# shenyunhang/APE

Hardware: AMD Instinct MI355X
Metric: images/sec @1024^2 APE-L_D fwd (higher is better)
Workload: dtype bf16

## Files before the change

ape_amd/csrc/select.hip:

```cpp
#include "common.h"
#include "../../include/ape_hip.h"

__device__ __forceinline__ bool iou_gt(const float4 a, const float4 b, float thr) {
  const float area_a = (a.z - a.x) * (a.w - a.y);
  const float area_b = (b.z - b.x) * (b.w - b.y);
  const float xx1 = fmaxf(a.x, b.x), yy1 = fmaxf(a.y, b.y);
  const float xx2 = fminf(a.z, b.z), yy2 = fminf(a.w, b.w);
  const float w = fmaxf(0.f, xx2 - xx1), h = fmaxf(0.f, yy2 - yy1);
  const float inter = w * h;
  return inter / (area_a + area_b - inter) > thr;
}

__global__ __launch_bounds__(64) void nms_mask_kernel(const float4* __restrict__ boxes, const int* __restrict__ groups, int n,
                                                      float thr, unsigned long long* __restrict__ mask, int nw) {
  __shared__ float4 cb[64];
  __shared__ int cg[64];
  const int rb = blockIdx.y, cbk = blockIdx.x, t = threadIdx.x;
  const int j0 = cbk * 64;
  if (j0 + t < n) {
    cb[t] = boxes[j0 + t];
    cg[t] = groups ? groups[j0 + t] : 0;
  }
  __syncthreads();
  const int i = rb * 64 + t;
  if (i >= n) return;
  const float4 bi = boxes[i];
  const int gi = groups ? groups[i] : 0;
  unsigned long long bits = 0ull;
  const int cnt = min(64, n - j0);
  for (int j = 0; j < cnt; ++j) {
    if (j0 + j != i && cg[j] == gi && iou_gt(bi, cb[j], thr)) bits |= (1ull << j);
  }
  mask[(size_t)i * nw + cbk] = bits;
}

__device__ __forceinline__ unsigned long long readlane64(unsigned long long v, int lane_uniform) {
  const unsigned lo = (unsigned)__builtin_amdgcn_readlane((int)(unsigned)(v & 0xffffffffull), lane_uniform);
  const unsigned hi = (unsigned)__builtin_amdgcn_readlane((int)(unsigned)(v >> 32), lane_uniform);
  return ((unsigned long long)hi << 32) | lo;
}

__device__ __forceinline__ unsigned long long uniform64(unsigned long long v) {
  const unsigned lo = (unsigned)__builtin_amdgcn_readfirstlane((int)(unsigned)(v & 0xffffffffull));
  const unsigned hi = (unsigned)__builtin_amdgcn_readfirstlane((int)(unsigned)(v >> 32));
  return ((unsigned long long)hi << 32) | lo;
}
__device__ __forceinline__ unsigned long long wave_or64(unsigned long long v) {
  unsigned lo = (unsigned)(v & 0xffffffffull), hi = (unsigned)(v >> 32);
#pragma unroll
  for (int o = 32; o > 0; o >>= 1) { lo |= (unsigned)__shfl_xor((int)lo, o, 64); hi |= (unsigned)__shfl_xor((int)hi, o, 64); }
  return ((unsigned long long)hi << 32) | lo;
}

template <bool USE_LDS>
__global__ __launch_bounds__(256) void nms_scan_segments_kernel(const unsigned long long* __restrict__ mask, int nw, int n,
                                                                const int* __restrict__ seg, const uint8_t* __restrict__ valid,
                                                                uint8_t* __restrict__ keep) {
  extern __shared__ __attribute__((aligned(16))) unsigned long long sub[];
  const int s0 = seg[blockIdx.x], s1 = seg[blockIdx.x + 1];
  if (s1 <= s0) return;
  const int w0 = s0 >> 6, w1 = (s1 - 1) >> 6;
  const int nws = w1 - w0 + 1;
  const int r_base = w0 * 64;
  if (USE_LDS) {
    const int nrows = (w1 + 1) * 64 - r_base;
    for (int e = threadIdx.x; e < nrows * nws; e += 256) {
      const int r = e / nws, w = e - r * nws;
      const int row = r_base + r;
      sub[e] = row < n ? mask[(size_t)row * nw + w0 + w] : 0ull;
    }
    __syncthreads();
  }
  if (threadIdx.x >= 64) return;
  const int lane = threadIdx.x;
  auto word = [&](int row, int c) -> unsigned long long {
    if (USE_LDS) return sub[(size_t)(row - r_base) * nws + (c - w0)];
    return mask[(size_t)(row < n ? row : n - 1) * nw + c];
  };
  unsigned long long kept0 = 0ull, kept1 = 0ull;
  for (int c = w0; c <= w1; ++c) {
    unsigned long long acc = 0ull;
    for (int cp = w0; cp < c; cp += 8) {
      unsigned long long t[8];
#pragma unroll
      for (int u = 0; u < 8; ++u) {
        const int cq = cp + u;
        const int cqc = cq < c ? cq : cp;
        const int rel = cqc - w0;
        const unsigned long long km = readlane64(rel >= 64 ? kept1 : kept0, rel & 63);
        const bool take = cq < c && ((km >> lane) & 1ull);
        const unsigned long long v = word(cqc * 64 + lane, c);
        t[u] = take ? v : 0ull;
      }
#pragma unroll
      for (int u = 0; u < 8; ++u) acc |= t[u];
    }
    const unsigned long long remc = uniform64(wave_or64(acc));
    const int i = c * 64 + lane;
    const bool in_seg = i >= s0 && i < s1;
    const bool ok = in_seg && (valid == nullptr || valid[i] != 0);
    const unsigned long long row_c = ok ? word(i, c) : 0ull;
    unsigned long long alive = __builtin_amdgcn_ballot_w64(ok) & ~remc;
    unsigned long long kept = 0ull;
    while (alive != 0ull) {
      const int j = __builtin_ctzll(alive);
      kept |= 1ull << j;
      alive &= ~(1ull << j);
      alive &= ~readlane64(row_c, j);
    }
    if (in_seg) keep[i] = (uint8_t)((kept >> lane) & 1ull);
    const int rel = c - w0;
    if (lane == (rel & 63)) { if (rel >= 64) kept1 = kept; else kept0 = kept; }
  }
}

__global__ __launch_bounds__(256) void nms_scan_classes_kernel(const unsigned long long* __restrict__ mask, int nw, int n,
                                                               const int* __restrict__ order, const uint8_t* __restrict__ valid,
                                                               uint8_t* __restrict__ keep, int num_classes) {
  extern __shared__ __attribute__((aligned(16))) unsigned long long smask[];
  const int tid = threadIdx.x, lane = tid & 63, wave = tid >> 6;
  for (int i = tid; i < n * nw; i += 256) smask[i] = mask[i];
  __syncthreads();
  const int c = blockIdx.x * 4 + wave;
  if (c >= num_classes) return;
  const int* ord = order + (size_t)c * n;
  unsigned long long rem = 0ull;
  for (int base = 0; base < n; base += 64) {
    const int p = base + lane;
    const int qv = p < n ? ord[p] : 0;
    const int okv = (p < n) && (valid == nullptr || valid[(size_t)c * n + p] != 0);
    int keptv = 0;
    const int cnt = min(64, n - base);
    for (int u = 0; u < cnt; ++u) {
      const int qi = __builtin_amdgcn_readlane(qv, u);
      const int ok = __builtin_amdgcn_readlane(okv, u);
      const unsigned long long row = lane < nw ? smask[(size_t)qi * nw + lane] : 0ull;
      const unsigned long long r = readlane64(rem, qi >> 6);
      const bool kept = ok && !((r >> (qi & 63)) & 1ull);
      if (kept) rem |= row;
      if (lane == u) keptv = kept ? 1 : 0;
    }
    if (p < n) keep[(size_t)c * n + p] = (uint8_t)keptv;
  }
}

extern "C" int ape_hip_nms_mask_words(int n) { return ceil_div(n, 64); }

extern "C" int ape_hip_nms_mask(const float* boxes, const int* groups, int n, float iou_thr, uint64_t* mask, void* stream) {
  APE_CHECK_ARG(boxes && mask && n > 0 && ((uintptr_t)boxes) % 16 == 0, "ape_hip_nms_mask: bad args");
  const int nw = ceil_div(n, 64);
  APE_LAUNCH(nms_mask_kernel, dim3(nw, nw), dim3(64), 0, (hipStream_t)stream, (const float4*)boxes, groups, n, iou_thr,
                     (unsigned long long*)mask, nw);
  APE_CHECK_LAUNCH("ape_hip_nms_mask");
  return 0;
}

extern "C" int ape_hip_nms_scan_segments(const uint64_t* mask, int n, const int* seg_offsets, int num_segments, int max_segment,
                                         const uint8_t* valid, uint8_t* keep, void* stream) {
  APE_CHECK_ARG(mask && seg_offsets && keep && n > 0 && num_segments > 0, "ape_hip_nms_scan_segments: bad args");
  APE_CHECK_ARG(max_segment <= 126 * 64, "ape_hip_nms_scan_segments: segment longer than %d candidates", 126 * 64);
  const size_t sub_rows = (size_t)(ceil_div(max_segment, 64) + 1) * 64, sub_words = (size_t)ceil_div(max_segment, 64) + 1;
  const size_t lds = sub_rows * sub_words * 8;
  if (lds <= 160 * 1024) {
    static ApeOncePerDevice attr_done;
    if (attr_done.first()) {
      (void)hipFuncSetAttribute((const void*)nms_scan_segments_kernel<true>, hipFuncAttributeMaxDynamicSharedMemorySize, 160 * 1024);
    }
    APE_LAUNCH(nms_scan_segments_kernel<true>, dim3(num_segments), dim3(256), lds, (hipStream_t)stream,
                       (const unsigned long long*)mask, ceil_div(n, 64), n, seg_offsets, valid, keep);
  } else {
    APE_LAUNCH(nms_scan_segments_kernel<false>, dim3(num_segments), dim3(256), 0, (hipStream_t)stream,
                       (const unsigned long long*)mask, ceil_div(n, 64), n, seg_offsets, valid, keep);
  }
  APE_CHECK_LAUNCH("ape_hip_nms_scan_segments");
  return 0;
}

extern "C" int ape_hip_nms_scan_classes(const uint64_t* mask, int n, const int* order, int num_classes, const uint8_t* valid,
                                        uint8_t* keep, void* stream) {
  const int nw = ceil_div(n, 64);
  const size_t lds = (size_t)n * nw * 8;
  APE_CHECK_ARG(mask && order && keep && n > 0 && num_classes > 0 && lds <= 160 * 1024,
                "ape_hip_nms_scan_classes: bad args (the n x n/64 bit matrix must fit the 160 KiB LDS: n <= 1280)");
  static ApeOncePerDevice attr_done;
  if (attr_done.first()) {
    (void)hipFuncSetAttribute((const void*)nms_scan_classes_kernel, hipFuncAttributeMaxDynamicSharedMemorySize, 160 * 1024);
  }
  APE_LAUNCH(nms_scan_classes_kernel, dim3(ceil_div(num_classes, 4)), dim3(256), lds, (hipStream_t)stream,
                     (const unsigned long long*)mask, nw, n, order, valid, keep, num_classes);
  APE_CHECK_LAUNCH("ape_hip_nms_scan_classes");
  return 0;
}
```

ape_amd/csrc/topk.hip:

```cpp
#include "common.h"
#include "../../include/ape_hip.h"

typedef unsigned long long u64;
#define TK_THREADS 1024

__device__ __forceinline__ uint32_t ordkey(float x) {
  const uint32_t u = __float_as_uint(x);
  return u ^ ((u >> 31) ? 0xffffffffu : 0x80000000u);
}
__device__ __forceinline__ float ordkey_inv(uint32_t k) {
  return __uint_as_float(k ^ ((k >> 31) ? 0x80000000u : 0xffffffffu));
}
__device__ __forceinline__ float sigmoid_f(float x) { return 1.f / (1.f + expf(-x)); }

struct TkLevels {
  int start[8];
  int n[8];
  int L;
};
__device__ __forceinline__ int level_of(const TkLevels& lv, int idx) {
  int l = 0;
#pragma unroll
  for (int i = 1; i < 8; ++i) l += (i < lv.L && idx >= lv.start[i]) ? 1 : 0;
  return l;
}

template <int N>
__device__ __forceinline__ void bitonic_desc(u64* s) {
  for (int k = 2; k <= N; k <<= 1) {
    for (int j = k >> 1; j > 0; j >>= 1) {
      for (int i = threadIdx.x; i < N; i += TK_THREADS) {
        const int p = i ^ j;
        if (p > i) {
          const u64 a = s[i], b = s[p];
          const bool first_larger = (i & k) == 0;
          if (first_larger ? (a < b) : (a > b)) { s[i] = b; s[p] = a; }
        }
      }
      __syncthreads();
    }
  }
}

template <typename KeyFn>
__device__ __forceinline__ void radix_select(KeyFn key, int n, int k, uint32_t* hist, uint32_t* sh, uint32_t& thr, uint32_t& rem) {
  uint32_t prefix = 0, r = (uint32_t)k;
  for (int shift = 24; shift >= 0; shift -= 8) {
    for (int b = threadIdx.x; b < 256; b += TK_THREADS) hist[b] = 0;
    __syncthreads();
    const uint32_t himask = shift == 24 ? 0u : (0xffffffffu << (shift + 8));
    for (int i0 = 0; i0 < n; i0 += TK_THREADS) {
      const int i = i0 + threadIdx.x;
      const uint32_t kk = i < n ? key(i) : 0u;
      bool live = i < n && (kk & himask) == prefix;
      const uint32_t bin = (kk >> shift) & 255u;
      u64 todo = __ballot(live);
      while (todo) {
        const int leader = __ffsll((long long)todo) - 1;
        const uint32_t lb = (uint32_t)__builtin_amdgcn_readlane((int)bin, leader);
        const u64 same = __ballot(live && bin == lb);
        if ((int)(threadIdx.x & 63) == leader) atomicAdd(&hist[lb], (uint32_t)__popcll(same));
        todo &= ~same;
        if (live && bin == lb) live = false;
      }
    }
    __syncthreads();
    if (threadIdx.x == 0) {
      uint32_t cum = 0;
      int b = 255;
      for (; b > 0; --b) {
        if (cum + hist[b] >= r) break;
        cum += hist[b];
      }
      sh[0] = prefix | ((uint32_t)b << shift);
      sh[1] = r - cum;
    }
    __syncthreads();
    prefix = sh[0];
    r = sh[1];
    __syncthreads();
  }
  thr = prefix;
  rem = r;
}

template <typename KeyFn, typename CompFn>
__device__ __forceinline__ void block_topk(KeyFn key, CompFn composite, int n, int k, u64* comp, uint32_t* hist, uint32_t* sh, uint32_t* wcnt) {
  comp[threadIdx.x] = 0ull;
  __syncthreads();
  if (n <= k) {
    for (int i = threadIdx.x; i < n; i += TK_THREADS) comp[i] = composite(i);
    __syncthreads();
  } else {
    uint32_t thr, rem;
    radix_select(key, n, k, hist, sh, thr, rem);
    const uint32_t ngt = (uint32_t)k - rem;
    const int lane = threadIdx.x & 63, wave = threadIdx.x >> 6;
    uint32_t base_gt = 0, base_eq = 0;
    for (int i0 = 0; i0 < n; i0 += TK_THREADS) {
      const int i = i0 + threadIdx.x;
      const uint32_t kk = i < n ? key(i) : 0u;
      const bool gt = i < n && kk > thr, eq = i < n && kk == thr;
      const u64 bg = __ballot(gt), be = __ballot(eq);
      const u64 lt = (1ull << lane) - 1ull;
      if (lane == 0) { wcnt[wave] = (uint32_t)__popcll(bg); wcnt[16 + wave] = (uint32_t)__popcll(be); }
      __syncthreads();
      uint32_t wg = 0, we = 0, tg = 0, te = 0;
#pragma unroll
      for (int w = 0; w < 16; ++w) {
        const uint32_t cg = wcnt[w], ce = wcnt[16 + w];
        if (w < wave) { wg += cg; we += ce; }
        tg += cg; te += ce;
      }
      if (gt) comp[base_gt + wg + (uint32_t)__popcll(bg & lt)] = composite(i);
      if (eq) {
        const uint32_t rank = base_eq + we + (uint32_t)__popcll(be & lt);
        if (rank < rem) comp[ngt + rank] = composite(i);
      }
      base_gt += tg;
      base_eq += te;
      __syncthreads();
    }
  }
  bitonic_desc<1024>(comp);
}

template <int PER>
__device__ __forceinline__ void block_topk_regs(const uint32_t (&kk)[PER], int n, int k, uint32_t gbase, u64* comp, uint32_t* hist,
                                                uint32_t* sh, uint32_t* wcnt) {
  comp[threadIdx.x] = 0ull;
  __syncthreads();
  const int lane = threadIdx.x & 63, wave = threadIdx.x >> 6;
  if (n <= k) {
    if ((int)threadIdx.x < n) comp[threadIdx.x] = ((u64)kk[0] << 32) | (u64)(0xffffffffu - (gbase + threadIdx.x));
    __syncthreads();
  } else {
    uint32_t prefix = 0, r = (uint32_t)k;
    for (int shift = 24; shift >= 0; shift -= 8) {
      for (int b = threadIdx.x; b < 256; b += TK_THREADS) hist[b] = 0;
      __syncthreads();
      const uint32_t himask = shift == 24 ? 0u : (0xffffffffu << (shift + 8));
#pragma unroll
      for (int j = 0; j < PER; ++j) {
        const int e = j * TK_THREADS + threadIdx.x;
        bool live = e < n && (kk[j] & himask) == prefix;
        const uint32_t bin = (kk[j] >> shift) & 255u;
        u64 todo = __ballot(live);
        while (todo) {
          const int leader = __ffsll((long long)todo) - 1;
          const uint32_t lb = (uint32_t)__builtin_amdgcn_readlane((int)bin, leader);
          const u64 same = __ballot(live && bin == lb);
          if (lane == leader) atomicAdd(&hist[lb], (uint32_t)__popcll(same));
          todo &= ~same;
          if (live && bin == lb) live = false;
        }
      }
      __syncthreads();
      if (threadIdx.x == 0) {
        uint32_t cum = 0;
        int b = 255;
        for (; b > 0; --b) {
          if (cum + hist[b] >= r) break;
          cum += hist[b];
        }
        sh[0] = prefix | ((uint32_t)b << shift);
        sh[1] = r - cum;
      }
      __syncthreads();
      prefix = sh[0];
      r = sh[1];
      __syncthreads();
    }
    const uint32_t thr = prefix, rem = r, ngt = (uint32_t)k - rem;
    uint32_t base_gt = 0, base_eq = 0;
#pragma unroll
    for (int j = 0; j < PER; ++j) {
      const int e = j * TK_THREADS + threadIdx.x;
      const bool gt = e < n && kk[j] > thr, eq = e < n && kk[j] == thr;
      const u64 bg = __ballot(gt), be = __ballot(eq);
      const u64 lt = (1ull << lane) - 1ull;
      if (lane == 0) { wcnt[wave] = (uint32_t)__popcll(bg); wcnt[16 + wave] = (uint32_t)__popcll(be); }
      __syncthreads();
      uint32_t wg = 0, we = 0, tg = 0, te = 0;
#pragma unroll
      for (int w = 0; w < 16; ++w) {
        const uint32_t cg = wcnt[w], ce = wcnt[16 + w];
        if (w < wave) { wg += cg; we += ce; }
        tg += cg; te += ce;
      }
      const u64 c = ((u64)kk[j] << 32) | (u64)(0xffffffffu - (gbase + (uint32_t)e));
      if (gt) comp[base_gt + wg + (uint32_t)__popcll(bg & lt)] = c;
      if (eq) {
        const uint32_t rank = base_eq + we + (uint32_t)__popcll(be & lt);
        if (rank < rem) comp[ngt + rank] = c;
      }
      base_gt += tg;
      base_eq += te;
      __syncthreads();
    }
  }
  bitonic_desc<1024>(comp);
}

#define TK_STAGE2_MAX 12288
#define TK_MAX_JOBS 96
struct TkJobs {
  int njobs, nseg;
  int seg_first[8], seg_jobs[8], seg_k[8], seg_n[8], seg_mode[8];
  int start[TK_MAX_JOBS], n[TK_MAX_JOBS], seg[TK_MAX_JOBS];
};

__device__ __forceinline__ void stage2_gather(const u64* __restrict__ ws, int first_job, int njobs, int k, u64* lds) {
  const int m = njobs * k;
  for (int i = threadIdx.x; i < m; i += TK_THREADS) lds[i] = ws[(size_t)(first_job + i / k) * 1024 + (i % k)];
  __syncthreads();
}

__global__ __launch_bounds__(256) void enc_finalize_kernel(const float* __restrict__ cls2, const float* __restrict__ d,
                                                           const float* __restrict__ anchors, int T, float* __restrict__ enc_class,
                                                           float* __restrict__ enc_coord, float* __restrict__ xyxy) {
  const int t = blockIdx.x * 256 + threadIdx.x;
  if (t >= T) return;
  const float2 c = *reinterpret_cast<const float2*>(cls2 + 2 * (size_t)t);
  const bool pick = c.y > c.x;
  enc_class[t] = pick ? c.y : c.x;
  const float4 dd = *reinterpret_cast<const float4*>(d + 8 * (size_t)t + (pick ? 4 : 0));
  const float4 a = *reinterpret_cast<const float4*>(anchors + 4 * (size_t)t);
  const float4 u = make_float4(dd.x + a.x, dd.y + a.y, dd.z + a.z, dd.w + a.w);
  *reinterpret_cast<float4*>(enc_coord + 4 * (size_t)t) = u;
  const float cx = sigmoid_f(u.x), cy = sigmoid_f(u.y), w = sigmoid_f(u.z), h = sigmoid_f(u.w);
  float4 b = make_float4(cx - 0.5f * w, cy - 0.5f * h, cx + 0.5f * w, cy + 0.5f * h);
  b.x = fminf(fmaxf(b.x, 0.f), 1.f); b.y = fminf(fmaxf(b.y, 0.f), 1.f);
  b.z = fminf(fmaxf(b.z, 0.f), 1.f); b.w = fminf(fmaxf(b.w, 0.f), 1.f);
  *reinterpret_cast<float4*>(xyxy + 4 * (size_t)t) = b;
}

template <int PER>
__global__ __launch_bounds__(TK_THREADS) void topk_stage1_kernel(const float* __restrict__ x, TkJobs jobs, u64* __restrict__ ws) {
  __shared__ u64 comp[1024];
  __shared__ uint32_t hist[256], sh[2], wcnt[32];
  const int job = blockIdx.x, seg = jobs.seg[job], start = jobs.start[job], n = jobs.n[job];
  const bool sig = jobs.seg_mode[seg] != 0;
  uint32_t kk[PER];
#pragma unroll
  for (int j = 0; j < PER; ++j) {
    const int e = j * TK_THREADS + threadIdx.x;
    const float v = e < n ? x[start + e] : 0.f;
    kk[j] = e < n ? ordkey(sig ? sigmoid_f(v) : v) : 0u;
  }
  block_topk_regs<PER>(kk, n, jobs.seg_k[seg], (uint32_t)start, comp, hist, sh, wcnt);
  ws[(size_t)job * 1024 + threadIdx.x] = comp[threadIdx.x];
}

__global__ __launch_bounds__(TK_THREADS) void proposal_topk2_kernel(const u64* __restrict__ ws, TkJobs jobs, TkLevels lv, int k, int k_alt,
                                                                    int32_t* __restrict__ cand, int32_t* __restrict__ alt) {
  extern __shared__ u64 lds[];
  __shared__ u64 comp[1024];
  __shared__ uint32_t hist[256], sh[2], wcnt[32];
  const int l = blockIdx.x;
  const int kk = jobs.seg_k[l], m = jobs.seg_jobs[l] * kk;
  stage2_gather(ws, jobs.seg_first[l], jobs.seg_jobs[l], kk, lds);
  auto key = [&](int i) { return (uint32_t)(lds[i] >> 32); };
  auto composite = [&](int i) { return lds[i]; };
  block_topk(key, composite, m, kk, comp, hist, sh, wcnt);
  if (l == lv.L) {
    for (int r = threadIdx.x; r < k_alt; r += TK_THREADS) alt[r] = (int32_t)(0xffffffffu - (uint32_t)(comp[r] & 0xffffffffull));
    return;
  }
  const int start = lv.start[l], n = lv.n[l];
  const int own = n < k ? n : k;
  for (int r = threadIdx.x; r < k; r += TK_THREADS) {
    int idx;
    if (r < own) {
      idx = (int)(0xffffffffu - (uint32_t)(comp[r] & 0xffffffffull));
    } else {
      const int e = r - n;
      idx = e >= start ? e + n : e;
    }
    cand[l * k + r] = idx;
  }
}

__device__ __forceinline__ void scan5(const uint32_t v[5], uint32_t out[5], uint32_t tot[5], u64* sa, uint32_t* sb) {
  const int lane = threadIdx.x & 63, wave = threadIdx.x >> 6;
  u64 a = (u64)v[0] | ((u64)v[1] << 16) | ((u64)v[2] << 32) | ((u64)v[3] << 48);
  uint32_t b = v[4];
  u64 ia = a;
  uint32_t ib = b;
#pragma unroll
  for (int o = 1; o < 64; o <<= 1) {
    const uint32_t lo = __shfl_up((uint32_t)(ia & 0xffffffffull), o, 64), hi = __shfl_up((uint32_t)(ia >> 32), o, 64);
    const uint32_t tb = __shfl_up(ib, o, 64);
    if (lane >= o) { ia += ((u64)hi << 32) | lo; ib += tb; }
  }
  __syncthreads();
  if (lane == 63) { sa[wave] = ia; sb[wave] = ib; }
  __syncthreads();
  u64 wa = 0, ta = 0;
  uint32_t wb = 0, tb2 = 0;
#pragma unroll
  for (int w = 0; w < 16; ++w) {
    if (w < wave) { wa += sa[w]; wb += sb[w]; }
    ta += sa[w]; tb2 += sb[w];
  }
  const u64 ea = wa + ia - a;
  out[0] = (uint32_t)(ea & 0xffff); out[1] = (uint32_t)((ea >> 16) & 0xffff); out[2] = (uint32_t)((ea >> 32) & 0xffff);
  out[3] = (uint32_t)((ea >> 48) & 0xffff); out[4] = wb + ib - b;
  tot[0] = (uint32_t)(ta & 0xffff); tot[1] = (uint32_t)((ta >> 16) & 0xffff); tot[2] = (uint32_t)((ta >> 32) & 0xffff);
  tot[3] = (uint32_t)((ta >> 48) & 0xffff); tot[4] = tb2;
}

#define PO_PAD 8192
#define PO_PER (PO_PAD / TK_THREADS)
__global__ __launch_bounds__(TK_THREADS) void proposal_order_kernel(const int32_t* __restrict__ cand, int n, const float* __restrict__ logit,
                                                                    const float* __restrict__ xyxy, TkLevels lv,
                                                                    float* __restrict__ boxes_b, int32_t* __restrict__ groups_b,
                                                                    int32_t* __restrict__ seg, int32_t* __restrict__ cand_a,
                                                                    int32_t* __restrict__ lv_a, int32_t* __restrict__ pos_b) {
  extern __shared__ u64 po_lds[];
  __shared__ u64 sa[16];
  __shared__ uint32_t sb[16];
  const int nchunks = (n + 1023) >> 10, npad = nchunks << 10;
  u64* work = po_lds;
  u64* srt = po_lds + npad;
  for (int p = threadIdx.x; p < npad; p += TK_THREADS)
    work[p] = p < n ? (((u64)ordkey(logit[cand[p]]) << 32) | (u64)(0xffffffffu - (uint32_t)p)) : (u64)(npad - 1 - p);
  __syncthreads();
  for (int k = 2; k <= 1024; k <<= 1) {
    for (int j = k >> 1; j > 0; j >>= 1) {
      for (int i = threadIdx.x; i < npad; i += TK_THREADS) {
        const int q = i ^ j;
        if (q > i) {
          const u64 a = work[i], b = work[q];
          const bool first_larger = ((i & 1023) & k) == 0;
          if (first_larger ? (a < b) : (a > b)) { work[i] = b; work[q] = a; }
        }
      }
      __syncthreads();
    }
  }
  for (int i = threadIdx.x; i < npad; i += TK_THREADS) {
    const u64 v = work[i];
    const int c = i >> 10;
    int rank = i & 1023;
    for (int o = 0; o < nchunks; ++o) {
      if (o == c) continue;
      const u64* ch = work + (o << 10);
      int lo = 0, hi = 1024;
      while (lo < hi) {
        const int mid = (lo + hi) >> 1;
        if (ch[mid] > v) lo = mid + 1; else hi = mid;
      }
      rank += lo;
    }
    srt[rank] = v;
  }
  __syncthreads();
  int idx[PO_PER], lev[PO_PER];
  uint32_t cnt[5] = {0, 0, 0, 0, 0};
#pragma unroll
  for (int j = 0; j < PO_PER; ++j) {
    const int a = threadIdx.x * PO_PER + j;
    idx[j] = -1; lev[j] = 0;
    if (a < n) {
      const int p = (int)(0xffffffffu - (uint32_t)(srt[a] & 0xffffffffull));
      idx[j] = cand[p];
      lev[j] = level_of(lv, idx[j]);
      cnt[lev[j]] += 1;
    }
  }
  uint32_t ex[5], tot[5];
  scan5(cnt, ex, tot, sa, sb);
  uint32_t segs[6];
  segs[0] = 0;
#pragma unroll
  for (int l = 0; l < 5; ++l) segs[l + 1] = segs[l] + tot[l];
  if (threadIdx.x == 0)
    for (int l = 0; l <= lv.L; ++l) seg[l] = (int32_t)segs[l];
#pragma unroll
  for (int j = 0; j < PO_PER; ++j) {
    const int a = threadIdx.x * PO_PER + j;
    if (a < n) {
      const int l = lev[j];
      const int b = (int)(segs[l] + ex[l]);
      ex[l] += 1;
      cand_a[a] = idx[j]; lv_a[a] = l; pos_b[a] = b;
      groups_b[b] = l;
      *reinterpret_cast<float4*>(boxes_b + 4 * (size_t)b) = *reinterpret_cast<const float4*>(xyxy + 4 * (size_t)idx[j]);
    }
  }
}

__global__ __launch_bounds__(TK_THREADS) void proposal_quota_kernel(const int32_t* __restrict__ cand_a, const int32_t* __restrict__ lv_a,
                                                                    const int32_t* __restrict__ pos_b, const uint8_t* __restrict__ keep_b,
                                                                    int n, const int32_t* __restrict__ alt, int n_alt, TkLevels lv, int nq,
                                                                    long long* __restrict__ out) {
  __shared__ u64 sa[16];
  __shared__ uint32_t sb[16];
  int X[PO_PER], lev[PO_PER];
  bool valid[PO_PER];
  uint32_t c[5] = {0, 0, 0, 0, 0};
#pragma unroll
  for (int j = 0; j < PO_PER; ++j) {
    const int a = threadIdx.x * PO_PER + j;
    X[j] = 0; lev[j] = 0; valid[j] = false;
    if (a < n) {
      X[j] = cand_a[a]; lev[j] = lv_a[a];
      valid[j] = keep_b[pos_b[a]] != 0;
      c[0] += valid[j] ? 1u : 0u;
    }
  }
  uint32_t ex[5], tot[5];
  scan5(c, ex, tot, sa, sb);
  const bool use_alt = (int)tot[0] < nq;
  if (use_alt) {
#pragma unroll
    for (int j = 0; j < PO_PER; ++j) {
      const int a = threadIdx.x * PO_PER + j;
      valid[j] = a < n && a < n_alt;
      X[j] = valid[j] ? alt[a] : 0;
      lev[j] = level_of(lv, X[j]);
    }
  }
  for (int r = threadIdx.x; r < nq; r += TK_THREADS) out[r] = 0;
#pragma unroll
  for (int l = 0; l < 5; ++l) c[l] = 0;
#pragma unroll
  for (int j = 0; j < PO_PER; ++j)
    if (valid[j]) c[lev[j]] += 1;
  scan5(c, ex, tot, sa, sb);
  const uint32_t quota = (uint32_t)(nq / lv.L);
  bool sel[PO_PER];
  uint32_t c2[5] = {0, 0, 0, 0, 0};
#pragma unroll
  for (int j = 0; j < PO_PER; ++j) {
    sel[j] = false;
    if (valid[j]) {
      sel[j] = ex[lev[j]] < quota;
      ex[lev[j]] += 1;
      c2[sel[j] ? 0 : 1] += 1;
    }
  }
  scan5(c2, ex, tot, sa, sb);
  const uint32_t need = (uint32_t)nq - tot[0];
  uint32_t c3[5] = {0, 0, 0, 0, 0};
  uint32_t rest = ex[1];
#pragma unroll
  for (int j = 0; j < PO_PER; ++j) {
    if (valid[j] && !sel[j]) {
      if (rest < need) sel[j] = true;
      rest += 1;
    }
    c3[0] += sel[j] ? 1u : 0u;
  }
  scan5(c3, ex, tot, sa, sb);
  uint32_t slot = ex[0];
#pragma unroll
  for (int j = 0; j < PO_PER; ++j)
    if (sel[j]) {
      if (slot < (uint32_t)nq) out[slot] = (long long)X[j];
      slot += 1;
    }
}

__global__ __launch_bounds__(64) void det_boxes_kernel(const float* __restrict__ logits, int ldl, int K, const float* __restrict__ boxes,
                                                       const float* __restrict__ scale, float* __restrict__ xyxy,
                                                       uint8_t* __restrict__ finite) {
  const int q = blockIdx.x, lane = threadIdx.x;
  bool ok = true;
  for (int c = lane; c < K; c += 64) ok = ok && isfinite(sigmoid_f(logits[(size_t)q * ldl + c]));
  ok = __ballot(!ok) == 0ull;
  if (lane == 0) {
    const float4 b = *reinterpret_cast<const float4*>(boxes + 4 * (size_t)q);
    const float4 s = *reinterpret_cast<const float4*>(scale);
    float4 o = make_float4((b.x - 0.5f * b.z) * s.x, (b.y - 0.5f * b.w) * s.y, (b.x + 0.5f * b.z) * s.z, (b.y + 0.5f * b.w) * s.w);
    ok = ok && isfinite(o.x) && isfinite(o.y) && isfinite(o.z) && isfinite(o.w);
    o.x = fminf(fmaxf(o.x, 0.f), s.x); o.y = fminf(fmaxf(o.y, 0.f), s.y);
    o.z = fminf(fmaxf(o.z, 0.f), s.z); o.w = fminf(fmaxf(o.w, 0.f), s.w);
    if (!ok) o = make_float4(0.f, 0.f, 0.f, 0.f);
    *reinterpret_cast<float4*>(xyxy + 4 * (size_t)q) = o;
    finite[q] = ok ? 1 : 0;
  }
}

__global__ __launch_bounds__(TK_THREADS) void class_sort_kernel(const float* __restrict__ logits, int ldl, int Q, const uint8_t* __restrict__ finite,
                                                                float thresh, float* __restrict__ sorted, int32_t* __restrict__ order,
                                                                uint8_t* __restrict__ valid) {
  __shared__ u64 comp[1024];
  const int c = blockIdx.x, q = threadIdx.x;
  comp[q] = q < Q ? (((u64)ordkey(sigmoid_f(logits[(size_t)q * ldl + c])) << 32) | (u64)(0xffffffffu - (uint32_t)q)) : 0ull;
  __syncthreads();
  bitonic_desc<1024>(comp);
  if (q < Q) {
    const float s = ordkey_inv((uint32_t)(comp[q] >> 32));
    const int src = (int)(0xffffffffu - (uint32_t)(comp[q] & 0xffffffffull));
    sorted[(size_t)c * Q + q] = s;
    order[(size_t)c * Q + q] = src;
    valid[(size_t)c * Q + q] = (s > thresh && finite[src]) ? 1 : 0;
  }
}

template <int PER>
__global__ __launch_bounds__(TK_THREADS) void det_topk1_kernel(const float* __restrict__ sorted, const uint8_t* __restrict__ keep, int total,
                                                               int k, u64* __restrict__ ws) {
  __shared__ u64 comp[1024];
  __shared__ uint32_t hist[256], sh[2], wcnt[32];
  const int start = blockIdx.x * (PER * TK_THREADS);
  const int n = min(PER * TK_THREADS, total - start);
  uint32_t kk[PER];
#pragma unroll
  for (int j = 0; j < PER; ++j) {
    const int e = j * TK_THREADS + threadIdx.x;
    kk[j] = e < n ? ordkey(keep[start + e] ? sorted[start + e] : -1.f) : 0u;
  }
  block_topk_regs<PER>(kk, n, k, (uint32_t)start, comp, hist, sh, wcnt);
  ws[(size_t)blockIdx.x * 1024 + threadIdx.x] = comp[threadIdx.x];
}

__global__ __launch_bounds__(TK_THREADS) void topk_merge_kernel(const u64* __restrict__ in, int nlists, int group, int k, u64* __restrict__ out) {
  extern __shared__ u64 lds[];
  __shared__ u64 comp[1024];
  __shared__ uint32_t hist[256], sh[2], wcnt[32];
  const int first = blockIdx.x * group;
  const int cnt = min(group, nlists - first);
  stage2_gather(in, first, cnt, k, lds);
  auto key = [&](int i) { return (uint32_t)(lds[i] >> 32); };
  auto composite = [&](int i) { return lds[i]; };
  block_topk(key, composite, cnt * k, k, comp, hist, sh, wcnt);
  out[(size_t)blockIdx.x * 1024 + threadIdx.x] = comp[threadIdx.x];
}

__global__ __launch_bounds__(TK_THREADS) void det_topk2_kernel(const u64* __restrict__ ws, int nchunks, const int32_t* __restrict__ order,
                                                               const float* __restrict__ xyxy, int Q, int k, float* __restrict__ det_boxes,
                                                               float* __restrict__ det_scores, long long* __restrict__ det_classes,
                                                               long long* __restrict__ det_query) {
  extern __shared__ u64 lds[];
  __shared__ u64 comp[1024];
  __shared__ uint32_t hist[256], sh[2], wcnt[32];
  stage2_gather(ws, 0, nchunks, k, lds);
  auto key = [&](int i) { return (uint32_t)(lds[i] >> 32); };
  auto composite = [&](int i) { return lds[i]; };
  block_topk(key, composite, nchunks * k, k, comp, hist, sh, wcnt);
  for (int r = threadIdx.x; r < k; r += TK_THREADS) {
    const int flat = (int)(0xffffffffu - (uint32_t)(comp[r] & 0xffffffffull));
    const int qi = order[flat];
    det_scores[r] = ordkey_inv((uint32_t)(comp[r] >> 32));
    det_classes[r] = (long long)(flat / Q);
    det_query[r] = (long long)qi;
    *reinterpret_cast<float4*>(det_boxes + 4 * (size_t)r) = *reinterpret_cast<const float4*>(xyxy + 4 * (size_t)qi);
  }
}

static int fill_levels(TkLevels& lv, const int* level_start, const int* level_n, int L) {
  APE_CHECK_ARG(level_start && level_n && L >= 1 && L <= 5, "proposal selection: 1 <= levels <= 5");
  for (int i = 0; i < 8; ++i) { lv.start[i] = i < L ? level_start[i] : 0x7fffffff; lv.n[i] = i < L ? level_n[i] : 0; }
  lv.L = L;
  return 0;
}

extern "C" int ape_hip_enc_finalize(const float* cls2, const float* d, const float* anchors, int T, float* enc_class, float* enc_coord,
                                    float* xyxy, void* stream) {
  APE_CHECK_ARG(cls2 && d && anchors && enc_class && enc_coord && xyxy && T > 0, "ape_hip_enc_finalize: bad arguments");
  APE_LAUNCH(enc_finalize_kernel, dim3(ceil_div(T, 256)), dim3(256), 0, (hipStream_t)stream, cls2, d, anchors, T, enc_class,
                     enc_coord, xyxy);
  APE_CHECK_LAUNCH("enc_finalize_kernel");
  return 0;
}

static int topk_per(const int* seg_n, const int* seg_k, int nseg) {
  const int pers[3] = {8, 32, 64};
  for (int pi = 0; pi < 3; ++pi) {
    bool ok = true;
    int jobs = 0;
    for (int s = 0; s < nseg; ++s) {
      const int c = ceil_div(seg_n[s], pers[pi] * TK_THREADS);
      ok = ok && (long long)c * seg_k[s] <= TK_STAGE2_MAX;
      jobs += c;
    }
    if (ok && jobs <= TK_MAX_JOBS) return pers[pi];
  }
  return 0;
}

static void set_stage2_attr() {
  static ApeOncePerDevice done;
  if (done.first()) {
    (void)hipFuncSetAttribute((const void*)proposal_topk2_kernel, hipFuncAttributeMaxDynamicSharedMemorySize, 112 * 1024);
    (void)hipFuncSetAttribute((const void*)det_topk2_kernel, hipFuncAttributeMaxDynamicSharedMemorySize, 112 * 1024);
    (void)hipFuncSetAttribute((const void*)topk_merge_kernel, hipFuncAttributeMaxDynamicSharedMemorySize, 112 * 1024);
  }
}

extern "C" int ape_hip_topk_workspace_words(int n_total) {
  const int det = ceil_div(n_total > 0 ? n_total : 1, 8 * TK_THREADS);
  const int lists = det > TK_MAX_JOBS ? det : TK_MAX_JOBS;
  return 1024 * (lists + lists / 2 + 1);
}

extern "C" int ape_hip_proposal_topk(const float* logit, int T, const int* level_start, const int* level_n, int L, int k, int k_alt,
                                     uint64_t* workspace, int32_t* cand, int32_t* alt, void* stream) {
  TkLevels lv;
  if (fill_levels(lv, level_start, level_n, L)) return -1;
  APE_CHECK_ARG(logit && workspace && cand && alt && T > 0 && k >= 1 && k <= 1024 && k_alt >= 1 && k_alt <= 1024 && k <= T && k_alt <= T,
                "ape_hip_proposal_topk: 1 <= k, k_alt <= min(1024, T)");
  int seg_n[8], seg_k[8];
  for (int l = 0; l < L; ++l) { seg_n[l] = level_n[l]; seg_k[l] = k; }
  seg_n[L] = T; seg_k[L] = k_alt;
  const int per = topk_per(seg_n, seg_k, L + 1);
  APE_CHECK_ARG(per > 0, "ape_hip_proposal_topk: %d tokens do not fit the two-stage selection", T);
  TkJobs jobs;
  memset(&jobs, 0, sizeof(jobs));
  jobs.nseg = L + 1;
  const int chunk = per * TK_THREADS;
  for (int s = 0; s <= L; ++s) {
    const int base = s < L ? level_start[s] : 0;
    jobs.seg_first[s] = jobs.njobs; jobs.seg_k[s] = seg_k[s]; jobs.seg_n[s] = seg_n[s]; jobs.seg_mode[s] = s < L ? 1 : 0;
    for (int c0 = 0; c0 < seg_n[s]; c0 += chunk) {
      jobs.start[jobs.njobs] = base + c0; jobs.n[jobs.njobs] = seg_n[s] - c0 < chunk ? seg_n[s] - c0 : chunk; jobs.seg[jobs.njobs] = s;
      ++jobs.njobs;
    }
    jobs.seg_jobs[s] = jobs.njobs - jobs.seg_first[s];
  }
  hipStream_t st = (hipStream_t)stream;
  u64* ws = reinterpret_cast<u64*>(workspace);
  if (per == 8) APE_LAUNCH(topk_stage1_kernel<8>, dim3(jobs.njobs), dim3(TK_THREADS), 0, st, logit, jobs, ws);
  else if (per == 32) APE_LAUNCH(topk_stage1_kernel<32>, dim3(jobs.njobs), dim3(TK_THREADS), 0, st, logit, jobs, ws);
  else APE_LAUNCH(topk_stage1_kernel<64>, dim3(jobs.njobs), dim3(TK_THREADS), 0, st, logit, jobs, ws);
  set_stage2_attr();
  int mmax = 0;
  for (int s = 0; s <= L; ++s) mmax = mmax > jobs.seg_jobs[s] * jobs.seg_k[s] ? mmax : jobs.seg_jobs[s] * jobs.seg_k[s];
  APE_LAUNCH(proposal_topk2_kernel, dim3(L + 1), dim3(TK_THREADS), (size_t)mmax * sizeof(u64), st, ws, jobs, lv, k, k_alt, cand, alt);
  APE_CHECK_LAUNCH("proposal_topk");
  return 0;
}

extern "C" int ape_hip_proposal_order(const int32_t* cand, int n, const float* logit, const float* xyxy, const int* level_start,
                                      const int* level_n, int L, float* boxes_b, int32_t* groups_b, int32_t* seg, int32_t* cand_a,
                                      int32_t* lv_a, int32_t* pos_b, void* stream) {
  TkLevels lv;
  if (fill_levels(lv, level_start, level_n, L)) return -1;
  APE_CHECK_ARG(cand && logit && xyxy && boxes_b && groups_b && seg && cand_a && lv_a && pos_b && n > 0 && n <= PO_PAD,
                "ape_hip_proposal_order: 1 <= n <= 8192 candidates");
  static ApeOncePerDevice attr_done;
  if (attr_done.first()) {
    (void)hipFuncSetAttribute((const void*)proposal_order_kernel, hipFuncAttributeMaxDynamicSharedMemorySize, 2 * PO_PAD * sizeof(u64));
  }
  APE_LAUNCH(proposal_order_kernel, dim3(1), dim3(TK_THREADS), (size_t)2 * ((n + 1023) / 1024) * 1024 * sizeof(u64), (hipStream_t)stream, cand, n, logit, xyxy, lv,
                     boxes_b, groups_b, seg, cand_a, lv_a, pos_b);
  APE_CHECK_LAUNCH("proposal_order_kernel");
  return 0;
}

extern "C" int ape_hip_proposal_quota(const int32_t* cand_a, const int32_t* lv_a, const int32_t* pos_b, const uint8_t* keep_b, int n,
                                      const int32_t* alt, int n_alt, const int* level_start, const int* level_n, int L, int nq,
                                      int64_t* out, void* stream) {
  TkLevels lv;
  if (fill_levels(lv, level_start, level_n, L)) return -1;
  APE_CHECK_ARG(cand_a && lv_a && pos_b && keep_b && alt && out && n > 0 && n <= PO_PAD && n_alt >= 0 && nq > 0,
                "ape_hip_proposal_quota: bad arguments (n <= 8192)");
  APE_LAUNCH(proposal_quota_kernel, dim3(1), dim3(TK_THREADS), 0, (hipStream_t)stream, cand_a, lv_a, pos_b, keep_b, n, alt, n_alt,
                     lv, nq, (long long*)out);
  APE_CHECK_LAUNCH("proposal_quota_kernel");
  return 0;
}

extern "C" int ape_hip_det_sort(const float* logits, int ldl, int Q, int K, const float* boxes, const float* scale, float thresh,
                                float* xyxy, uint8_t* finite, float* sorted, int32_t* order, uint8_t* valid, void* stream) {
  APE_CHECK_ARG(logits && boxes && scale && xyxy && finite && sorted && order && valid && K > 0, "ape_hip_det_sort: bad arguments");
  APE_CHECK_ARG(Q > 0 && Q <= 1024, "ape_hip_det_sort: 1 <= queries <= 1024 (got %d)", Q);
  hipStream_t st = (hipStream_t)stream;
  APE_LAUNCH(det_boxes_kernel, dim3(Q), dim3(64), 0, st, logits, ldl, K, boxes, scale, xyxy, finite);
  APE_LAUNCH(class_sort_kernel, dim3(K), dim3(TK_THREADS), 0, st, logits, ldl, Q, finite, thresh, sorted, order, valid);
  APE_CHECK_LAUNCH("ape_hip_det_sort");
  return 0;
}

extern "C" int ape_hip_det_topk(const float* sorted, const uint8_t* keep, const int32_t* order, const float* xyxy, int K, int Q, int k,
                                uint64_t* workspace, float* det_boxes, float* det_scores, int64_t* det_classes, int64_t* det_query,
                                void* stream) {
  APE_CHECK_ARG(sorted && keep && order && xyxy && workspace && det_boxes && det_scores && det_classes && det_query, "ape_hip_det_topk: null pointer");
  APE_CHECK_ARG(K > 0 && Q > 0 && (long long)K * Q < 0x7fffffffLL && k >= 1 && k <= 1024 && k <= K * Q, "ape_hip_det_topk: 1 <= k <= min(1024, K*Q)");
  const int total = K * Q;
  int per = topk_per(&total, &k, 1);
  const bool merge = per == 0;
  if (merge) per = 64;
  int nchunks = ceil_div(total, per * TK_THREADS);
  hipStream_t st = (hipStream_t)stream;
  u64* ws = reinterpret_cast<u64*>(workspace);
  if (per == 8) APE_LAUNCH(det_topk1_kernel<8>, dim3(nchunks), dim3(TK_THREADS), 0, st, sorted, keep, total, k, ws);
  else if (per == 32) APE_LAUNCH(det_topk1_kernel<32>, dim3(nchunks), dim3(TK_THREADS), 0, st, sorted, keep, total, k, ws);
  else APE_LAUNCH(det_topk1_kernel<64>, dim3(nchunks), dim3(TK_THREADS), 0, st, sorted, keep, total, k, ws);
  set_stage2_attr();
  if (merge) {
    const int cap_lists = ape_hip_topk_workspace_words(total) / 1024;
    u64* a = ws;
    u64* b = ws + (size_t)1024 * (cap_lists - (cap_lists / 3));
    const int group = TK_STAGE2_MAX / k;
    while ((long long)nchunks * k > TK_STAGE2_MAX) {
      const int nout = ceil_div(nchunks, group);
      APE_LAUNCH(topk_merge_kernel, dim3(nout), dim3(TK_THREADS), (size_t)group * k * sizeof(u64), st, a, nchunks, group, k, b);
      u64* t = a; a = b; b = t;
      nchunks = nout;
    }
    ws = a;
  }
  APE_LAUNCH(det_topk2_kernel, dim3(1), dim3(TK_THREADS), (size_t)nchunks * k * sizeof(u64), st, ws, nchunks, order, xyxy, Q, k,
                     det_boxes, det_scores, (long long*)det_classes, (long long*)det_query);
  APE_CHECK_LAUNCH("det_topk");
  return 0;
}
```

ape_amd/csrc/vlpool.hip:

```cpp
#include "common.h"
#include "../../include/ape_hip.h"

#define VL_CHUNK 128
#define VL_H 8

__global__ __launch_bounds__(256) void vl_smax_partial_kernel(const float* __restrict__ S, int lds, int T, float* __restrict__ pmax) {
  __shared__ float sh[256];
  const int t = threadIdx.x, h = t & 7;
  const int base = blockIdx.x * VL_CHUNK;
  float m = -INFINITY;
  for (int k = 0; k < VL_CHUNK / 32; ++k) {
    const int tok = base + k * 32 + (t >> 3);
    if (tok < T) m = fmaxf(m, S[(size_t)tok * lds + h]);
  }
  sh[t] = m;
  __syncthreads();
  if (t < VL_H) {
    float a = -INFINITY;
    for (int j = t; j < 256; j += 8) a = fmaxf(a, sh[j]);
    pmax[blockIdx.x * VL_H + t] = a;
  }
}

template <typename TX>
__global__ __launch_bounds__(256) void vl_pool_partial_kernel(const float* __restrict__ S, int lds, const TX* __restrict__ x, int ldx,
                                                              int T, int C, const float* __restrict__ pmax, int nchunk,
                                                              float* __restrict__ pacc, float* __restrict__ psum) {
  __shared__ float hmax[VL_H];
  __shared__ float gmax_s;
  __shared__ float P[VL_CHUNK][VL_H];
  const int t = threadIdx.x;
  {
    float a = -INFINITY;
    for (int k = t >> 3; k < nchunk; k += 32) a = fmaxf(a, pmax[k * VL_H + (t & 7)]);
    P[t >> 3][t & 7] = a;
    __syncthreads();
    if (t < VL_H) {
      float m = -INFINITY;
      for (int j = 0; j < 32; ++j) m = fmaxf(m, P[j][t]);
      hmax[t] = m;
    }
  }
  __syncthreads();
  if (t == 0) {
    float g = hmax[0];
    for (int h = 1; h < VL_H; ++h) g = fmaxf(g, hmax[h]);
    gmax_s = g;
  }
  __syncthreads();
  const float gmax = gmax_s;
  const int base = blockIdx.x * VL_CHUNK;
  const int cnt = min(VL_CHUNK, T - base);
  for (int idx = t; idx < VL_CHUNK * VL_H; idx += 256) {
    const int r = idx >> 3, h = idx & 7;
    float p = 0.f;
    if (r < cnt) {
      float a = S[(size_t)(base + r) * lds + h] - gmax;
      a = fminf(fmaxf(a, -50000.f), 50000.f);
      const float mh = fminf(fmaxf(hmax[h] - gmax, -50000.f), 50000.f);
      float b = a - mh;
      b = fminf(fmaxf(b, -50000.f), 50000.f);
      p = expf(b);
    }
    P[r][h] = p;
  }
  __syncthreads();
  if (t < VL_H) {
    float s = 0.f;
    for (int r = 0; r < cnt; ++r) s += P[r][t];
    psum[blockIdx.x * VL_H + t] = s;
  }
  for (int c = t; c < C; c += 256) {
    float acc[VL_H];
#pragma unroll
    for (int h = 0; h < VL_H; ++h) acc[h] = 0.f;
    for (int r = 0; r < cnt; ++r) {
      const float xv = ldf<TX>(x + (size_t)(base + r) * ldx + c);
#pragma unroll
      for (int h = 0; h < VL_H; ++h) acc[h] = fmaf(P[r][h], xv, acc[h]);
    }
#pragma unroll
    for (int h = 0; h < VL_H; ++h) pacc[((size_t)blockIdx.x * VL_H + h) * C + c] = acc[h];
  }
}

__global__ __launch_bounds__(256) void vl_pool_final_kernel(const float* __restrict__ pacc, const float* __restrict__ psum, int nchunk,
                                                            int C, const float* __restrict__ sub, float* __restrict__ out) {
  __shared__ float sa[8][32];
  __shared__ float sl[256];
  const int h = blockIdx.x, t = threadIdx.x;
  const int kg = t >> 5, cl = t & 31;
  const int c = blockIdx.y * 32 + cl;
  float l = 0.f;
  for (int k = t; k < nchunk; k += 256) l += psum[k * VL_H + h];
  sl[t] = l;
  float a = 0.f;
  if (c < C) for (int k = kg; k < nchunk; k += 8) a += pacc[((size_t)k * VL_H + h) * C + c];
  sa[kg][cl] = a;
  __syncthreads();
  for (int o = 128; o > 0; o >>= 1) { if (t < o) sl[t] += sl[t + o]; __syncthreads(); }
  if (t < 32 && c < C) {
    float acc = 0.f;
#pragma unroll
    for (int g = 0; g < 8; ++g) acc += sa[g][t];
    out[h * C + c] = acc / sl[0] - (sub != nullptr ? sub[c] : 0.f);
  }
}

extern "C" int ape_hip_vl_pool_workspace_floats(int T, int C) {
  const int nchunk = ceil_div(T, VL_CHUNK);
  return nchunk * VL_H * (C + 2);
}

extern "C" int ape_hip_vl_pool(const float* S, int lds, const void* x, int ldx, int x_dt, int T, int C, float* workspace,
                               const float* sub, float* out, void* stream) {
  APE_CHECK_ARG(S && x && workspace && out && T > 0 && C > 0, "ape_hip_vl_pool: bad args");
  const int nchunk = ceil_div(T, VL_CHUNK);
  float* pmax = workspace;
  float* psum = pmax + nchunk * VL_H;
  float* pacc = psum + nchunk * VL_H;
  hipStream_t s = (hipStream_t)stream;
  APE_LAUNCH(vl_smax_partial_kernel, dim3(nchunk), dim3(256), 0, s, S, lds, T, pmax);
  if (x_dt == APE_DT_F16) APE_LAUNCH(vl_pool_partial_kernel<f16_t>, dim3(nchunk), dim3(256), 0, s, S, lds, (const f16_t*)x, ldx, T, C, pmax, nchunk, pacc, psum);
  else if (x_dt == APE_DT_BF16) APE_LAUNCH(vl_pool_partial_kernel<bf16_t>, dim3(nchunk), dim3(256), 0, s, S, lds, (const bf16_t*)x, ldx, T, C, pmax, nchunk, pacc, psum);
  else
    APE_LAUNCH(vl_pool_partial_kernel<float>, dim3(nchunk), dim3(256), 0, s, S, lds, (const float*)x, ldx, T, C, pmax, nchunk, pacc, psum);
  APE_LAUNCH(vl_pool_final_kernel, dim3(VL_H, ceil_div(C, 32)), dim3(256), 0, s, pacc, psum, nchunk, C, sub, out);
  APE_CHECK_LAUNCH("ape_hip_vl_pool");
  return 0;
}


template <typename TC>
__global__ __launch_bounds__(256) void head_gemv_kernel(const float* __restrict__ x, int ldx, const float* __restrict__ W,
                                                        const float* __restrict__ bias, float* __restrict__ out, int ldo, int H,
                                                        int N, int D, float alpha, TC* __restrict__ out_bf16, int ldob) {
  const int lane = threadIdx.x & 63;
  const int row = blockIdx.x * 4 + (threadIdx.x >> 6);
  if (row >= H * N) return;
  const int h = row / N, n = row % N;
  const float* w = W + (size_t)row * D;
  const float* xr = x + (size_t)h * ldx;
  float s = 0.f;
  if ((D & 3) == 0 && (ldx & 3) == 0) {
    for (int d = lane * 4; d < D; d += 256) {
      const float4 a = *reinterpret_cast<const float4*>(w + d), b = *reinterpret_cast<const float4*>(xr + d);
      s = fmaf(a.x, b.x, s); s = fmaf(a.y, b.y, s); s = fmaf(a.z, b.z, s); s = fmaf(a.w, b.w, s);
    }
  } else {
    for (int d = lane; d < D; d += 64) s = fmaf(w[d], xr[d], s);
  }
  s = wave_sum(s);
  if (lane == 0) {
    const float r = s * alpha + (bias != nullptr ? bias[row] : 0.f);
    out[(size_t)h * ldo + n] = r;
    if (out_bf16 != nullptr) stf<TC>(out_bf16 + (size_t)h * ldob + n, r);
  }
}

extern "C" int ape_hip_head_gemv(const float* x, int ldx, const float* W, const float* bias, float* out, int ldo, int H, int N,
                                 int D, float alpha, void* out_bf16, int ldob, int copy_dt, void* stream) {
  APE_CHECK_ARG(x && W && out && H > 0 && N > 0 && D > 0, "ape_hip_head_gemv: bad args");
  APE_CHECK_ARG(out_bf16 == nullptr || ape_is16(copy_dt), "ape_hip_head_gemv: the copy is bf16 or f16 (copy_dt %d)", copy_dt);
  APE_CHECK_ARG(((uintptr_t)x) % 16 == 0 && ((uintptr_t)W) % 16 == 0, "ape_hip_head_gemv: x / W must be 16-byte aligned");
  if (out_bf16 != nullptr && copy_dt == APE_DT_F16)
    APE_LAUNCH(head_gemv_kernel<f16_t>, dim3(ceil_div(H * N, 4)), dim3(256), 0, (hipStream_t)stream, x, ldx, W, bias, out, ldo, H, N, D, alpha,
                       (f16_t*)out_bf16, ldob);
  else
    APE_LAUNCH(head_gemv_kernel<bf16_t>, dim3(ceil_div(H * N, 4)), dim3(256), 0, (hipStream_t)stream, x, ldx, W, bias, out, ldo, H, N, D, alpha,
                       (bf16_t*)out_bf16, ldob);
  APE_CHECK_LAUNCH("ape_hip_head_gemv");
  return 0;
}
```

Before: 117.8.

## Rework top-k, NMS scan and VL-pool final kernels for wider parallelism

Several postprocessing kernels are reworked together. The bitonic sort now keeps values in registers, using wave shuffles for strides under 64 and double-buffered LDS only for larger strides. The radix select uses per-digit histograms with a wave-level scan pick instead of a single-thread loop, and top-k compaction computes per-wave counts once instead of syncing every chunk. The NMS segment scan stages its mask into LDS with 1024 threads and 16-byte loads, and the VL-pool final kernel uses narrower blocks with more loads in flight. These changes target sync-heavy, latency-bound small kernels on the detection postprocess path, but they add alignment requirements and enlarge the LDS footprint of the top-k kernels.

After: 118.9, median of 6. About the same (+0.9%).

```diff
diff --git a/ape_amd/csrc/select.hip b/ape_amd/csrc/select.hip
--- a/ape_amd/csrc/select.hip
+++ b/ape_amd/csrc/select.hip
@@ -52,22 +52,45 @@
   return ((unsigned long long)hi << 32) | lo;
 }
 
-template <bool USE_LDS>
-__global__ __launch_bounds__(256) void nms_scan_segments_kernel(const unsigned long long* __restrict__ mask, int nw, int n,
+#define NMS_SEG_THREADS 1024
+__global__ __launch_bounds__(NMS_SEG_THREADS) void nms_scan_segments_kernel(const unsigned long long* __restrict__ mask, int nw, int n,
                                                                 const int* __restrict__ seg, const uint8_t* __restrict__ valid,
-                                                                uint8_t* __restrict__ keep) {
+                                                                uint8_t* __restrict__ keep, int lds_words) {
   extern __shared__ __attribute__((aligned(16))) unsigned long long sub[];
   const int s0 = seg[blockIdx.x], s1 = seg[blockIdx.x + 1];
   if (s1 <= s0) return;
   const int w0 = s0 >> 6, w1 = (s1 - 1) >> 6;
   const int nws = w1 - w0 + 1;
   const int r_base = w0 * 64;
+  const int nrows = (w1 + 1) * 64 - r_base;
+  const bool USE_LDS = (long long)nrows * nws <= (long long)lds_words;
   if (USE_LDS) {
-    const int nrows = (w1 + 1) * 64 - r_base;
-    for (int e = threadIdx.x; e < nrows * nws; e += 256) {
-      const int r = e / nws, w = e - r * nws;
+    const int pl = threadIdx.x & 15;
+    const long long total = (long long)n * nw;
+#pragma unroll 4
+    for (int r = threadIdx.x >> 4; r < nrows; r += (int)(blockDim.x >> 4)) {
       const int row = r_base + r;
-      sub[e] = row < n ? mask[(size_t)row * nw + w0 + w] : 0ull;
+      unsigned long long* dst = sub + (size_t)r * nws;
+      if (row >= n) {
+        for (int w = pl; w < nws; w += 16) dst[w] = 0ull;
+        continue;
+      }
+      const long long g0 = (long long)row * nw + w0;
+      const long long a0 = g0 & ~1ll;
+      const int skew = (int)(g0 - a0);
+      for (int p = pl; 2 * p < nws + skew; p += 16) {
+        const long long a = a0 + 2 * p;
+        const int w = 2 * p - skew;
+        unsigned long long lo, hi = 0ull;
+        if (a + 1 < total) {
+          const ulonglong2 t = *reinterpret_cast<const ulonglong2*>(mask + a);
+          lo = t.x; hi = t.y;
+        } else {
+          lo = mask[a];
+        }
+        if (w >= 0) dst[w] = lo;
+        if (w + 1 < nws) dst[w + 1] = hi;
+      }
     }
     __syncthreads();
   }
@@ -119,7 +142,14 @@
                                                                uint8_t* __restrict__ keep, int num_classes) {
   extern __shared__ __attribute__((aligned(16))) unsigned long long smask[];
   const int tid = threadIdx.x, lane = tid & 63, wave = tid >> 6;
-  for (int i = tid; i < n * nw; i += 256) smask[i] = mask[i];
+  {
+    const int words = n * nw, pairs = words >> 1;
+    const ulonglong2* src = reinterpret_cast<const ulonglong2*>(mask);
+    ulonglong2* dst = reinterpret_cast<ulonglong2*>(smask);
+#pragma unroll 8
+    for (int i = tid; i < pairs; i += 256) dst[i] = src[i];
+    if ((words & 1) && tid == 0) smask[words - 1] = mask[words - 1];
+  }
   __syncthreads();
   const int c = blockIdx.x * 4 + wave;
   if (c >= num_classes) return;
@@ -159,19 +189,16 @@
                                          const uint8_t* valid, uint8_t* keep, void* stream) {
   APE_CHECK_ARG(mask && seg_offsets && keep && n > 0 && num_segments > 0, "ape_hip_nms_scan_segments: bad args");
   APE_CHECK_ARG(max_segment <= 126 * 64, "ape_hip_nms_scan_segments: segment longer than %d candidates", 126 * 64);
+  APE_CHECK_ARG(((uintptr_t)mask) % 16 == 0, "ape_hip_nms_scan_segments: mask must be 16-byte aligned");
   const size_t sub_rows = (size_t)(ceil_div(max_segment, 64) + 1) * 64, sub_words = (size_t)ceil_div(max_segment, 64) + 1;
-  const size_t lds = sub_rows * sub_words * 8;
-  if (lds <= 160 * 1024) {
-    static ApeOncePerDevice attr_done;
-    if (attr_done.first()) {
-      (void)hipFuncSetAttribute((const void*)nms_scan_segments_kernel<true>, hipFuncAttributeMaxDynamicSharedMemorySize, 160 * 1024);
-    }
-    APE_LAUNCH(nms_scan_segments_kernel<true>, dim3(num_segments), dim3(256), lds, (hipStream_t)stream,
-                       (const unsigned long long*)mask, ceil_div(n, 64), n, seg_offsets, valid, keep);
-  } else {
-    APE_LAUNCH(nms_scan_segments_kernel<false>, dim3(num_segments), dim3(256), 0, (hipStream_t)stream,
-                       (const unsigned long long*)mask, ceil_div(n, 64), n, seg_offsets, valid, keep);
-  }
+  size_t lds = sub_rows * sub_words * 8;
+  if (lds > 160 * 1024) lds = 0;
+  static ApeOncePerDevice attr_done;
+  if (attr_done.first()) {
+    (void)hipFuncSetAttribute((const void*)nms_scan_segments_kernel, hipFuncAttributeMaxDynamicSharedMemorySize, 160 * 1024);
+  }
+  APE_LAUNCH(nms_scan_segments_kernel, dim3(num_segments), dim3(lds ? NMS_SEG_THREADS : 256), lds, (hipStream_t)stream,
+                     (const unsigned long long*)mask, ceil_div(n, 64), n, seg_offsets, valid, keep, (int)(lds / 8));
   APE_CHECK_LAUNCH("ape_hip_nms_scan_segments");
   return 0;
 }
@@ -182,6 +209,7 @@
   const size_t lds = (size_t)n * nw * 8;
   APE_CHECK_ARG(mask && order && keep && n > 0 && num_classes > 0 && lds <= 160 * 1024,
                 "ape_hip_nms_scan_classes: bad args (the n x n/64 bit matrix must fit the 160 KiB LDS: n <= 1280)");
+  APE_CHECK_ARG(((uintptr_t)mask) % 16 == 0, "ape_hip_nms_scan_classes: mask must be 16-byte aligned");
   static ApeOncePerDevice attr_done;
   if (attr_done.first()) {
     (void)hipFuncSetAttribute((const void*)nms_scan_classes_kernel, hipFuncAttributeMaxDynamicSharedMemorySize, 160 * 1024);
diff --git a/ape_amd/csrc/topk.hip b/ape_amd/csrc/topk.hip
--- a/ape_amd/csrc/topk.hip
+++ b/ape_amd/csrc/topk.hip
@@ -25,181 +25,212 @@
   return l;
 }
 
-template <int N>
-__device__ __forceinline__ void bitonic_desc(u64* s) {
-  for (int k = 2; k <= N; k <<= 1) {
+__device__ __forceinline__ u64 shfl_xor64(u64 v, int m) {
+  const uint32_t lo = (uint32_t)__shfl_xor((int)(uint32_t)(v & 0xffffffffull), m, 64);
+  const uint32_t hi = (uint32_t)__shfl_xor((int)(uint32_t)(v >> 32), m, 64);
+  return ((u64)hi << 32) | lo;
+}
+
+template <int NV>
+__device__ __forceinline__ void bitonic_desc_regs(u64 (&v)[NV], int nv, u64* bufa, u64* bufb) {
+  const int i = threadIdx.x;
+  u64* buf = bufa;
+  u64* nxt = bufb;
+  for (int k = 2; k <= 1024; k <<= 1) {
+    const bool desc = (i & k) == 0;
     for (int j = k >> 1; j > 0; j >>= 1) {
-      for (int i = threadIdx.x; i < N; i += TK_THREADS) {
-        const int p = i ^ j;
-        if (p > i) {
-          const u64 a = s[i], b = s[p];
-          const bool first_larger = (i & k) == 0;
-          if (first_larger ? (a < b) : (a > b)) { s[i] = b; s[p] = a; }
-        }
+      const bool take_max = ((i & j) == 0) == desc;
+      if (j >= 64) {
+#pragma unroll
+        for (int c = 0; c < NV; ++c)
+          if (c < nv) buf[(c << 10) + i] = v[c];
+        __syncthreads();
+#pragma unroll
+        for (int c = 0; c < NV; ++c)
+          if (c < nv) {
+            const u64 o = buf[(c << 10) + (i ^ j)];
+            v[c] = ((v[c] > o) == take_max) ? v[c] : o;
+          }
+        u64* t = buf; buf = nxt; nxt = t;
+      } else {
+#pragma unroll
+        for (int c = 0; c < NV; ++c)
+          if (c < nv) {
+            const u64 o = shfl_xor64(v[c], j);
+            v[c] = ((v[c] > o) == take_max) ? v[c] : o;
+          }
+      }
+    }
+  }
+}
+
+__device__ __forceinline__ u64 sort_comp(u64* comp) {
+  u64 v[1] = {comp[threadIdx.x]};
+  bitonic_desc_regs<1>(v, 1, comp, comp + 1024);
+  comp[threadIdx.x] = v[0];
+  __syncthreads();
+  return v[0];
+}
+
+__device__ __forceinline__ void hist_add(uint32_t* hist, bool live, uint32_t bin) {
+  const u64 m = __ballot(live);
+  if (m == 0ull) return;
+  const int leader = __builtin_ctzll(m);
+  const uint32_t lb = (uint32_t)__builtin_amdgcn_readlane((int)bin, leader);
+  const u64 same = __ballot(live && bin == lb);
+  if (same == m) {
+    if ((int)(threadIdx.x & 63) == leader) atomicAdd(&hist[lb], (uint32_t)__popcll(m));
+  } else if (live) {
+    atomicAdd(&hist[bin], 1u);
+  }
+}
+__device__ __forceinline__ void hist_pick(const uint32_t* hist, int shift, uint32_t& prefix, uint32_t& r) {
+  const int lane = threadIdx.x & 63;
+  const int g = 63 - lane;
+  const uint4 h = *reinterpret_cast<const uint4*>(hist + 4 * g);
+  const uint32_t t = h.x + h.y + h.z + h.w;
+  uint32_t inc = t;
+#pragma unroll
+  for (int o = 1; o < 64; o <<= 1) {
+    const uint32_t u = (uint32_t)__shfl_up((int)inc, o, 64);
+    if (lane >= o) inc += u;
+  }
+  const u64 hit = __ballot(inc >= r);
+  const int src = hit ? __builtin_ctzll(hit) : 63;
+  uint32_t cum = inc - t;
+  int b = 0;
+  if (cum + h.w >= r) b = 3;
+  else {
+    cum += h.w;
+    if (cum + h.z >= r) b = 2;
+    else {
+      cum += h.z;
+      if (cum + h.y >= r) b = 1;
+      else cum += h.y;
+    }
+  }
+  b += 4 * g;
+  const uint32_t bu = (uint32_t)__builtin_amdgcn_readlane(b, src);
+  const uint32_t cu = (uint32_t)__builtin_amdgcn_readlane((int)cum, src);
+  prefix |= bu << shift;
+  r -= cu;
+}
+__device__ __forceinline__ void hist_clear(uint32_t* hist) { hist[threadIdx.x] = 0u; }
+
+__device__ __forceinline__ int tk_elem(int per, int j) { return (((int)(threadIdx.x >> 6) * per + j) << 6) + (int)(threadIdx.x & 63); }
+
+template <typename KeyFn, typename CompFn>
+__device__ __forceinline__ u64 block_topk(KeyFn key, CompFn composite, int n, int k, u64* comp, uint32_t* hist, uint32_t* wcnt) {
+  comp[threadIdx.x] = 0ull;
+  hist_clear(hist);
+  __syncthreads();
+  if (n <= k) {
+    for (int i = threadIdx.x; i < n; i += TK_THREADS) comp[i] = composite(i);
+  } else {
+    const int per = (n + TK_THREADS - 1) / TK_THREADS;
+    const int lane = threadIdx.x & 63, wave = threadIdx.x >> 6;
+    uint32_t prefix = 0, r = (uint32_t)k;
+    for (int d = 0; d < 4; ++d) {
+      const int shift = 24 - 8 * d;
+      const uint32_t himask = d == 0 ? 0u : (0xffffffffu << (shift + 8));
+      for (int j = 0; j < per; ++j) {
+        const int i = tk_elem(per, j);
+        const uint32_t kk = i < n ? key(i) : 0u;
+        hist_add(hist + 256 * d, i < n && (kk & himask) == prefix, (kk >> shift) & 255u);
       }
       __syncthreads();
-    }
-  }
-}
-
-template <typename KeyFn>
-__device__ __forceinline__ void radix_select(KeyFn key, int n, int k, uint32_t* hist, uint32_t* sh, uint32_t& thr, uint32_t& rem) {
-  uint32_t prefix = 0, r = (uint32_t)k;
-  for (int shift = 24; shift >= 0; shift -= 8) {
-    for (int b = threadIdx.x; b < 256; b += TK_THREADS) hist[b] = 0;
+      hist_pick(hist + 256 * d, shift, prefix, r);
+    }
+    const uint32_t thr = prefix, rem = r, ngt = (uint32_t)k - rem;
+    uint32_t cg = 0, ce = 0;
+    for (int j = 0; j < per; ++j) {
+      const int i = tk_elem(per, j);
+      const uint32_t kk = i < n ? key(i) : 0u;
+      cg += (uint32_t)__popcll(__ballot(i < n && kk > thr));
+      ce += (uint32_t)__popcll(__ballot(i < n && kk == thr));
+    }
+    if (lane == 0) { wcnt[wave] = cg; wcnt[16 + wave] = ce; }
     __syncthreads();
-    const uint32_t himask = shift == 24 ? 0u : (0xffffffffu << (shift + 8));
-    for (int i0 = 0; i0 < n; i0 += TK_THREADS) {
-      const int i = i0 + threadIdx.x;
-      const uint32_t kk = i < n ? key(i) : 0u;
-      bool live = i < n && (kk & himask) == prefix;
-      const uint32_t bin = (kk >> shift) & 255u;
-      u64 todo = __ballot(live);
-      while (todo) {
-        const int leader = __ffsll((long long)todo) - 1;
-        const uint32_t lb = (uint32_t)__builtin_amdgcn_readlane((int)bin, leader);
-        const u64 same = __ballot(live && bin == lb);
-        if ((int)(threadIdx.x & 63) == leader) atomicAdd(&hist[lb], (uint32_t)__popcll(same));
-        todo &= ~same;
-        if (live && bin == lb) live = false;
-      }
-    }
-    __syncthreads();
-    if (threadIdx.x == 0) {
-      uint32_t cum = 0;
-      int b = 255;
-      for (; b > 0; --b) {
-        if (cum + hist[b] >= r) break;
-        cum += hist[b];
-      }
-      sh[0] = prefix | ((uint32_t)b << shift);
-      sh[1] = r - cum;
-    }
-    __syncthreads();
-    prefix = sh[0];
-    r = sh[1];
-    __syncthreads();
-  }
-  thr = prefix;
-  rem = r;
-}
-
-template <typename KeyFn, typename CompFn>
-__device__ __forceinline__ void block_topk(KeyFn key, CompFn composite, int n, int k, u64* comp, uint32_t* hist, uint32_t* sh, uint32_t* wcnt) {
-  comp[threadIdx.x] = 0ull;
-  __syncthreads();
-  if (n <= k) {
-    for (int i = threadIdx.x; i < n; i += TK_THREADS) comp[i] = composite(i);
-    __syncthreads();
-  } else {
-    uint32_t thr, rem;
-    radix_select(key, n, k, hist, sh, thr, rem);
-    const uint32_t ngt = (uint32_t)k - rem;
-    const int lane = threadIdx.x & 63, wave = threadIdx.x >> 6;
     uint32_t base_gt = 0, base_eq = 0;
-    for (int i0 = 0; i0 < n; i0 += TK_THREADS) {
-      const int i = i0 + threadIdx.x;
+#pragma unroll
+    for (int w = 0; w < 16; ++w)
+      if (w < wave) { base_gt += wcnt[w]; base_eq += wcnt[16 + w]; }
+    const u64 lt = (1ull << lane) - 1ull;
+    for (int j = 0; j < per; ++j) {
+      const int i = tk_elem(per, j);
       const uint32_t kk = i < n ? key(i) : 0u;
       const bool gt = i < n && kk > thr, eq = i < n && kk == thr;
       const u64 bg = __ballot(gt), be = __ballot(eq);
-      const u64 lt = (1ull << lane) - 1ull;
-      if (lane == 0) { wcnt[wave] = (uint32_t)__popcll(bg); wcnt[16 + wave] = (uint32_t)__popcll(be); }
-      __syncthreads();
-      uint32_t wg = 0, we = 0, tg = 0, te = 0;
-#pragma unroll
-      for (int w = 0; w < 16; ++w) {
-        const uint32_t cg = wcnt[w], ce = wcnt[16 + w];
-        if (w < wave) { wg += cg; we += ce; }
-        tg += cg; te += ce;
-      }
-      if (gt) comp[base_gt + wg + (uint32_t)__popcll(bg & lt)] = composite(i);
+      if (gt) comp[base_gt + (uint32_t)__popcll(bg & lt)] = composite(i);
       if (eq) {
-        const uint32_t rank = base_eq + we + (uint32_t)__popcll(be & lt);
+        const uint32_t rank = base_eq + (uint32_t)__popcll(be & lt);
         if (rank < rem) comp[ngt + rank] = composite(i);
       }
-      base_gt += tg;
-      base_eq += te;
-      __syncthreads();
-    }
-  }
-  bitonic_desc<1024>(comp);
+      base_gt += (uint32_t)__popcll(bg);
+      base_eq += (uint32_t)__popcll(be);
+    }
+  }
+  __syncthreads();
+  return sort_comp(comp);
 }
 
 template <int PER>
-__device__ __forceinline__ void block_topk_regs(const uint32_t (&kk)[PER], int n, int k, uint32_t gbase, u64* comp, uint32_t* hist,
-                                                uint32_t* sh, uint32_t* wcnt) {
+__device__ __forceinline__ u64 block_topk_regs(const uint32_t (&kk)[PER], int n, int k, uint32_t gbase, u64* comp, uint32_t* hist,
+                                               uint32_t* wcnt) {
   comp[threadIdx.x] = 0ull;
+  hist_clear(hist);
   __syncthreads();
   const int lane = threadIdx.x & 63, wave = threadIdx.x >> 6;
   if (n <= k) {
-    if ((int)threadIdx.x < n) comp[threadIdx.x] = ((u64)kk[0] << 32) | (u64)(0xffffffffu - (gbase + threadIdx.x));
-    __syncthreads();
+#pragma unroll
+    for (int j = 0; j < PER; ++j) {
+      const int e = tk_elem(PER, j);
+      if (e < n) comp[e] = ((u64)kk[j] << 32) | (u64)(0xffffffffu - (gbase + (uint32_t)e));
+    }
   } else {
     uint32_t prefix = 0, r = (uint32_t)k;
-    for (int shift = 24; shift >= 0; shift -= 8) {
-      for (int b = threadIdx.x; b < 256; b += TK_THREADS) hist[b] = 0;
+#pragma unroll 1
+    for (int d = 0; d < 4; ++d) {
+      const int shift = 24 - 8 * d;
+      const uint32_t himask = d == 0 ? 0u : (0xffffffffu << (shift + 8));
+#pragma unroll
+      for (int j = 0; j < PER; ++j)
+        hist_add(hist + 256 * d, tk_elem(PER, j) < n && (kk[j] & himask) == prefix, (kk[j] >> shift) & 255u);
       __syncthreads();
-      const uint32_t himask = shift == 24 ? 0u : (0xffffffffu << (shift + 8));
-#pragma unroll
-      for (int j = 0; j < PER; ++j) {
-        const int e = j * TK_THREADS + threadIdx.x;
-        bool live = e < n && (kk[j] & himask) == prefix;
-        const uint32_t bin = (kk[j] >> shift) & 255u;
-        u64 todo = __ballot(live);
-        while (todo) {
-          const int leader = __ffsll((long long)todo) - 1;
-          const uint32_t lb = (uint32_t)__builtin_amdgcn_readlane((int)bin, leader);
-          const u64 same = __ballot(live && bin == lb);
-          if (lane == leader) atomicAdd(&hist[lb], (uint32_t)__popcll(same));
-          todo &= ~same;
-          if (live && bin == lb) live = false;
-        }
-      }
-      __syncthreads();
-      if (threadIdx.x == 0) {
-        uint32_t cum = 0;
-        int b = 255;
-        for (; b > 0; --b) {
-          if (cum + hist[b] >= r) break;
-          cum += hist[b];
-        }
-        sh[0] = prefix | ((uint32_t)b << shift);
-        sh[1] = r - cum;
-      }
-      __syncthreads();
-      prefix = sh[0];
-      r = sh[1];
-      __syncthreads();
+      hist_pick(hist + 256 * d, shift, prefix, r);
     }
     const uint32_t thr = prefix, rem = r, ngt = (uint32_t)k - rem;
+    uint32_t cg = 0, ce = 0;
+#pragma unroll
+    for (int j = 0; j < PER; ++j) {
+      const bool in = tk_elem(PER, j) < n;
+      cg += (uint32_t)__popcll(__ballot(in && kk[j] > thr));
+      ce += (uint32_t)__popcll(__ballot(in && kk[j] == thr));
+    }
+    if (lane == 0) { wcnt[wave] = cg; wcnt[16 + wave] = ce; }
+    __syncthreads();
     uint32_t base_gt = 0, base_eq = 0;
 #pragma unroll
+    for (int w = 0; w < 16; ++w)
+      if (w < wave) { base_gt += wcnt[w]; base_eq += wcnt[16 + w]; }
+    const u64 lt = (1ull << lane) - 1ull;
+#pragma unroll
     for (int j = 0; j < PER; ++j) {
-      const int e = j * TK_THREADS + threadIdx.x;
+      const int e = tk_elem(PER, j);
       const bool gt = e < n && kk[j] > thr, eq = e < n && kk[j] == thr;
       const u64 bg = __ballot(gt), be = __ballot(eq);
-      const u64 lt = (1ull << lane) - 1ull;
-      if (lane == 0) { wcnt[wave] = (uint32_t)__popcll(bg); wcnt[16 + wave] = (uint32_t)__popcll(be); }
-      __syncthreads();
-      uint32_t wg = 0, we = 0, tg = 0, te = 0;
-#pragma unroll
-      for (int w = 0; w < 16; ++w) {
-        const uint32_t cg = wcnt[w], ce = wcnt[16 + w];
-        if (w < wave) { wg += cg; we += ce; }
-        tg += cg; te += ce;
-      }
       const u64 c = ((u64)kk[j] << 32) | (u64)(0xffffffffu - (gbase + (uint32_t)e));
-      if (gt) comp[base_gt + wg + (uint32_t)__popcll(bg & lt)] = c;
+      if (gt) comp[base_gt + (uint32_t)__popcll(bg & lt)] = c;
       if (eq) {
-        const uint32_t rank = base_eq + we + (uint32_t)__popcll(be & lt);
+        const uint32_t rank = base_eq + (uint32_t)__popcll(be & lt);
         if (rank < rem) comp[ngt + rank] = c;
       }
-      base_gt += tg;
-      base_eq += te;
-      __syncthreads();
-    }
-  }
-  bitonic_desc<1024>(comp);
+      base_gt += (uint32_t)__popcll(bg);
+      base_eq += (uint32_t)__popcll(be);
+    }
+  }
+  __syncthreads();
+  return sort_comp(comp);
 }
 
 #define TK_STAGE2_MAX 12288
@@ -211,8 +242,8 @@
 };
 
 __device__ __forceinline__ void stage2_gather(const u64* __restrict__ ws, int first_job, int njobs, int k, u64* lds) {
-  const int m = njobs * k;
-  for (int i = threadIdx.x; i < m; i += TK_THREADS) lds[i] = ws[(size_t)(first_job + i / k) * 1024 + (i % k)];
+  for (int l = 0; l < njobs; ++l)
+    for (int r = threadIdx.x; r < k; r += TK_THREADS) lds[l * k + r] = ws[(size_t)(first_job + l) * 1024 + r];
   __syncthreads();
 }
 
@@ -237,32 +268,33 @@
 
 template <int PER>
 __global__ __launch_bounds__(TK_THREADS) void topk_stage1_kernel(const float* __restrict__ x, TkJobs jobs, u64* __restrict__ ws) {
-  __shared__ u64 comp[1024];
-  __shared__ uint32_t hist[256], sh[2], wcnt[32];
+  __shared__ u64 comp[2048];
+  __shared__ __attribute__((aligned(16))) uint32_t hist[1024];
+  __shared__ uint32_t wcnt[32];
   const int job = blockIdx.x, seg = jobs.seg[job], start = jobs.start[job], n = jobs.n[job];
   const bool sig = jobs.seg_mode[seg] != 0;
   uint32_t kk[PER];
 #pragma unroll
   for (int j = 0; j < PER; ++j) {
-    const int e = j * TK_THREADS + threadIdx.x;
+    const int e = tk_elem(PER, j);
     const float v = e < n ? x[start + e] : 0.f;
     kk[j] = e < n ? ordkey(sig ? sigmoid_f(v) : v) : 0u;
   }
-  block_topk_regs<PER>(kk, n, jobs.seg_k[seg], (uint32_t)start, comp, hist, sh, wcnt);
-  ws[(size_t)job * 1024 + threadIdx.x] = comp[threadIdx.x];
+  ws[(size_t)job * 1024 + threadIdx.x] = block_topk_regs<PER>(kk, n, jobs.seg_k[seg], (uint32_t)start, comp, hist, wcnt);
 }
 
 __global__ __launch_bounds__(TK_THREADS) void proposal_topk2_kernel(const u64* __restrict__ ws, TkJobs jobs, TkLevels lv, int k, int k_alt,
                                                                     int32_t* __restrict__ cand, int32_t* __restrict__ alt) {
   extern __shared__ u64 lds[];
-  __shared__ u64 comp[1024];
-  __shared__ uint32_t hist[256], sh[2], wcnt[32];
+  __shared__ u64 comp[2048];
+  __shared__ __attribute__((aligned(16))) uint32_t hist[1024];
+  __shared__ uint32_t wcnt[32];
   const int l = blockIdx.x;
   const int kk = jobs.seg_k[l], m = jobs.seg_jobs[l] * kk;
   stage2_gather(ws, jobs.seg_first[l], jobs.seg_jobs[l], kk, lds);
   auto key = [&](int i) { return (uint32_t)(lds[i] >> 32); };
   auto composite = [&](int i) { return lds[i]; };
-  block_topk(key, composite, m, kk, comp, hist, sh, wcnt);
+  block_topk(key, composite, m, kk, comp, hist, wcnt);
   if (l == lv.L) {
     for (int r = threadIdx.x; r < k_alt; r += TK_THREADS) alt[r] = (int32_t)(0xffffffffu - (uint32_t)(comp[r] & 0xffffffffull));
     return;
@@ -323,37 +355,34 @@
   const int nchunks = (n + 1023) >> 10, npad = nchunks << 10;
   u64* work = po_lds;
   u64* srt = po_lds + npad;
-  for (int p = threadIdx.x; p < npad; p += TK_THREADS)
-    work[p] = p < n ? (((u64)ordkey(logit[cand[p]]) << 32) | (u64)(0xffffffffu - (uint32_t)p)) : (u64)(npad - 1 - p);
-  __syncthreads();
-  for (int k = 2; k <= 1024; k <<= 1) {
-    for (int j = k >> 1; j > 0; j >>= 1) {
-      for (int i = threadIdx.x; i < npad; i += TK_THREADS) {
-        const int q = i ^ j;
-        if (q > i) {
-          const u64 a = work[i], b = work[q];
-          const bool first_larger = ((i & 1023) & k) == 0;
-          if (first_larger ? (a < b) : (a > b)) { work[i] = b; work[q] = a; }
-        }
-      }
-      __syncthreads();
-    }
-  }
-  for (int i = threadIdx.x; i < npad; i += TK_THREADS) {
-    const u64 v = work[i];
-    const int c = i >> 10;
-    int rank = i & 1023;
-    for (int o = 0; o < nchunks; ++o) {
-      if (o == c) continue;
-      const u64* ch = work + (o << 10);
-      int lo = 0, hi = 1024;
-      while (lo < hi) {
-        const int mid = (lo + hi) >> 1;
-        if (ch[mid] > v) lo = mid + 1; else hi = mid;
-      }
-      rank += lo;
-    }
-    srt[rank] = v;
+  u64 v[PO_PER];
+#pragma unroll
+  for (int c = 0; c < PO_PER; ++c) {
+    const int p = (c << 10) + threadIdx.x;
+    v[c] = 0ull;
+    if (c < nchunks) v[c] = p < n ? (((u64)ordkey(logit[cand[p]]) << 32) | (u64)(0xffffffffu - (uint32_t)p)) : (u64)(npad - 1 - p);
+  }
+  bitonic_desc_regs<PO_PER>(v, nchunks, work, srt);
+#pragma unroll
+  for (int c = 0; c < PO_PER; ++c)
+    if (c < nchunks) work[(c << 10) + threadIdx.x] = v[c];
+  __syncthreads();
+#pragma unroll
+  for (int c = 0; c < PO_PER; ++c) {
+    if (c >= nchunks) continue;
+    int pos[PO_PER];
+#pragma unroll
+    for (int o = 0; o < PO_PER; ++o) pos[o] = 0;
+    for (int s = 512; s > 0; s >>= 1) {
+#pragma unroll
+      for (int o = 0; o < PO_PER; ++o)
+        if (o != c && o < nchunks && work[(o << 10) + pos[o] + s - 1] > v[c]) pos[o] += s;
+    }
+    int rank = threadIdx.x;
+#pragma unroll
+    for (int o = 0; o < PO_PER; ++o)
+      if (o != c && o < nchunks) rank += pos[o] + (work[(o << 10) + pos[o]] > v[c] ? 1 : 0);
+    srt[rank] = v[c];
   }
   __syncthreads();
   int idx[PO_PER], lev[PO_PER];
@@ -486,14 +515,13 @@
 __global__ __launch_bounds__(TK_THREADS) void class_sort_kernel(const float* __restrict__ logits, int ldl, int Q, const uint8_t* __restrict__ finite,
                                                                 float thresh, float* __restrict__ sorted, int32_t* __restrict__ order,
                                                                 uint8_t* __restrict__ valid) {
-  __shared__ u64 comp[1024];
+  __shared__ u64 xbuf[2048];
   const int c = blockIdx.x, q = threadIdx.x;
-  comp[q] = q < Q ? (((u64)ordkey(sigmoid_f(logits[(size_t)q * ldl + c])) << 32) | (u64)(0xffffffffu - (uint32_t)q)) : 0ull;
-  __syncthreads();
-  bitonic_desc<1024>(comp);
+  u64 v[1] = {q < Q ? (((u64)ordkey(sigmoid_f(logits[(size_t)q * ldl + c])) << 32) | (u64)(0xffffffffu - (uint32_t)q)) : 0ull};
+  bitonic_desc_regs<1>(v, 1, xbuf, xbuf + 1024);
   if (q < Q) {
-    const float s = ordkey_inv((uint32_t)(comp[q] >> 32));
-    const int src = (int)(0xffffffffu - (uint32_t)(comp[q] & 0xffffffffull));
+    const float s = ordkey_inv((uint32_t)(v[0] >> 32));
+    const int src = (int)(0xffffffffu - (uint32_t)(v[0] & 0xffffffffull));
     sorted[(size_t)c * Q + q] = s;
     order[(size_t)c * Q + q] = src;
     valid[(size_t)c * Q + q] = (s > thresh && finite[src]) ? 1 : 0;
@@ -503,31 +531,31 @@
 template <int PER>
 __global__ __launch_bounds__(TK_THREADS) void det_topk1_kernel(const float* __restrict__ sorted, const uint8_t* __restrict__ keep, int total,
                                                                int k, u64* __restrict__ ws) {
-  __shared__ u64 comp[1024];
-  __shared__ uint32_t hist[256], sh[2], wcnt[32];
+  __shared__ u64 comp[2048];
+  __shared__ __attribute__((aligned(16))) uint32_t hist[1024];
+  __shared__ uint32_t wcnt[32];
   const int start = blockIdx.x * (PER * TK_THREADS);
   const int n = min(PER * TK_THREADS, total - start);
   uint32_t kk[PER];
 #pragma unroll
   for (int j = 0; j < PER; ++j) {
-    const int e = j * TK_THREADS + threadIdx.x;
+    const int e = tk_elem(PER, j);
     kk[j] = e < n ? ordkey(keep[start + e] ? sorted[start + e] : -1.f) : 0u;
   }
-  block_topk_regs<PER>(kk, n, k, (uint32_t)start, comp, hist, sh, wcnt);
-  ws[(size_t)blockIdx.x * 1024 + threadIdx.x] = comp[threadIdx.x];
+  ws[(size_t)blockIdx.x * 1024 + threadIdx.x] = block_topk_regs<PER>(kk, n, k, (uint32_t)start, comp, hist, wcnt);
 }
 
 __global__ __launch_bounds__(TK_THREADS) void topk_merge_kernel(const u64* __restrict__ in, int nlists, int group, int k, u64* __restrict__ out) {
   extern __shared__ u64 lds[];
-  __shared__ u64 comp[1024];
-  __shared__ uint32_t hist[256], sh[2], wcnt[32];
+  __shared__ u64 comp[2048];
+  __shared__ __attribute__((aligned(16))) uint32_t hist[1024];
+  __shared__ uint32_t wcnt[32];
   const int first = blockIdx.x * group;
   const int cnt = min(group, nlists - first);
   stage2_gather(in, first, cnt, k, lds);
   auto key = [&](int i) { return (uint32_t)(lds[i] >> 32); };
   auto composite = [&](int i) { return lds[i]; };
-  block_topk(key, composite, cnt * k, k, comp, hist, sh, wcnt);
-  out[(size_t)blockIdx.x * 1024 + threadIdx.x] = comp[threadIdx.x];
+  out[(size_t)blockIdx.x * 1024 + threadIdx.x] = block_topk(key, composite, cnt * k, k, comp, hist, wcnt);
 }
 
 __global__ __launch_bounds__(TK_THREADS) void det_topk2_kernel(const u64* __restrict__ ws, int nchunks, const int32_t* __restrict__ order,
@@ -535,12 +563,13 @@
                                                                float* __restrict__ det_scores, long long* __restrict__ det_classes,
                                                                long long* __restrict__ det_query) {
   extern __shared__ u64 lds[];
-  __shared__ u64 comp[1024];
-  __shared__ uint32_t hist[256], sh[2], wcnt[32];
+  __shared__ u64 comp[2048];
+  __shared__ __attribute__((aligned(16))) uint32_t hist[1024];
+  __shared__ uint32_t wcnt[32];
   stage2_gather(ws, 0, nchunks, k, lds);
   auto key = [&](int i) { return (uint32_t)(lds[i] >> 32); };
   auto composite = [&](int i) { return lds[i]; };
-  block_topk(key, composite, nchunks * k, k, comp, hist, sh, wcnt);
+  block_topk(key, composite, nchunks * k, k, comp, hist, wcnt);
   for (int r = threadIdx.x; r < k; r += TK_THREADS) {
     const int flat = (int)(0xffffffffu - (uint32_t)(comp[r] & 0xffffffffull));
     const int qi = order[flat];
diff --git a/ape_amd/csrc/vlpool.hip b/ape_amd/csrc/vlpool.hip
--- a/ape_amd/csrc/vlpool.hip
+++ b/ape_amd/csrc/vlpool.hip
@@ -9,6 +9,7 @@
   const int t = threadIdx.x, h = t & 7;
   const int base = blockIdx.x * VL_CHUNK;
   float m = -INFINITY;
+#pragma unroll
   for (int k = 0; k < VL_CHUNK / 32; ++k) {
     const int tok = base + k * 32 + (t >> 3);
     if (tok < T) m = fmaxf(m, S[(size_t)tok * lds + h]);
@@ -84,22 +85,43 @@
   }
 }
 
-__global__ __launch_bounds__(256) void vl_pool_final_kernel(const float* __restrict__ pacc, const float* __restrict__ psum, int nchunk,
-                                                            int C, const float* __restrict__ sub, float* __restrict__ out) {
-  __shared__ float sa[8][32];
+#define VL_FIN_COLS 16
+#define VL_FIN_IN_FLIGHT 16
+__global__ __launch_bounds__(8 * VL_FIN_COLS) void vl_pool_final_kernel(const float* __restrict__ pacc, const float* __restrict__ psum,
+                                                                        int nchunk, int C, const float* __restrict__ sub,
+                                                                        float* __restrict__ out) {
+  __shared__ float sa[8][VL_FIN_COLS];
   __shared__ float sl[256];
+  constexpr int NT = 8 * VL_FIN_COLS;
   const int h = blockIdx.x, t = threadIdx.x;
-  const int kg = t >> 5, cl = t & 31;
-  const int c = blockIdx.y * 32 + cl;
-  float l = 0.f;
-  for (int k = t; k < nchunk; k += 256) l += psum[k * VL_H + h];
-  sl[t] = l;
+  const int kg = t / VL_FIN_COLS, cl = t % VL_FIN_COLS;
+  const int c = blockIdx.y * VL_FIN_COLS + cl;
+  for (int j = t; j < 256; j += NT) {
+    float l = 0.f;
+    for (int k = j; k < nchunk; k += 256) l += psum[k * VL_H + h];
+    sl[j] = l;
+  }
   float a = 0.f;
-  if (c < C) for (int k = kg; k < nchunk; k += 8) a += pacc[((size_t)k * VL_H + h) * C + c];
+  if (c < C) {
+    const float* src = pacc + (size_t)h * C + c;
+    const size_t step = (size_t)VL_H * C;
+    int k = kg;
+    for (; k + 8 * (VL_FIN_IN_FLIGHT - 1) < nchunk; k += 8 * VL_FIN_IN_FLIGHT) {
+      float v[VL_FIN_IN_FLIGHT];
+#pragma unroll
+      for (int u = 0; u < VL_FIN_IN_FLIGHT; ++u) v[u] = src[(size_t)(k + 8 * u) * step];
+#pragma unroll
+      for (int u = 0; u < VL_FIN_IN_FLIGHT; ++u) a += v[u];
+    }
+    for (; k < nchunk; k += 8) a += src[(size_t)k * step];
+  }
   sa[kg][cl] = a;
   __syncthreads();
-  for (int o = 128; o > 0; o >>= 1) { if (t < o) sl[t] += sl[t + o]; __syncthreads(); }
-  if (t < 32 && c < C) {
+  for (int o = 128; o > 0; o >>= 1) {
+    for (int j = t; j < o; j += NT) sl[j] += sl[j + o];
+    __syncthreads();
+  }
+  if (t < VL_FIN_COLS && c < C) {
     float acc = 0.f;
 #pragma unroll
     for (int g = 0; g < 8; ++g) acc += sa[g][t];
@@ -125,7 +147,7 @@
   else if (x_dt == APE_DT_BF16) APE_LAUNCH(vl_pool_partial_kernel<bf16_t>, dim3(nchunk), dim3(256), 0, s, S, lds, (const bf16_t*)x, ldx, T, C, pmax, nchunk, pacc, psum);
   else
     APE_LAUNCH(vl_pool_partial_kernel<float>, dim3(nchunk), dim3(256), 0, s, S, lds, (const float*)x, ldx, T, C, pmax, nchunk, pacc, psum);
-  APE_LAUNCH(vl_pool_final_kernel, dim3(VL_H, ceil_div(C, 32)), dim3(256), 0, s, pacc, psum, nchunk, C, sub, out);
+  APE_LAUNCH(vl_pool_final_kernel, dim3(VL_H, ceil_div(C, VL_FIN_COLS)), dim3(8 * VL_FIN_COLS), 0, s, pacc, psum, nchunk, C, sub, out);
   APE_CHECK_LAUNCH("ape_hip_vl_pool");
   return 0;
 }
```
